# evanwporter/SparseCholesky

Hardware: AMD Instinct MI355X
Metric: numeric-factorization fp64 GFLOP/s (F=sum colcount^2) (higher is better)
Workload: dtype f64

## Files before the change

### sparsecholesky_amd/csrc/kernels.hip

```cpp
#include <hip/hip_runtime.h>

#include <cstdint>
#include <type_traits>

#include "kernels.hpp"

namespace sc {

typedef double double4_t __attribute__((ext_vector_type(4)));

__device__ __forceinline__ void report_fail(int32_t* info, const int32_t* post, int32_t col_internal) {
    atomicMin(info, (post ? post[col_internal] : col_internal) + 1);
}

__device__ __forceinline__ int bnd_at(const int32_t* b, int k, int mbc) {
    const int klo = b[0], khi = b[1];
    return k <= klo ? b[2] : (k >= khi ? mbc : b[2 + k - klo]);
}

__device__ __forceinline__ int lower_bound_i32(const int32_t* a, int n, int v) {
    int lo = 0, hi = n;
    while (lo < hi) {
        int mid = (lo + hi) >> 1;
        if (a[mid] < v)
// ... 947 lines not shown
        if (has_parent) {
            put(i + 1);
            take();
            if (i + 2 < count) prefetch(i + 2);
        }
        if (stamp && tid == 0) stamp[2] = __builtin_amdgcn_s_memtime();
        small_steps<1>(R, colbuf, w, P.info, P.post, d.c0);
        if (w == 0) lds_barrier();
        if (stamp && tid == 0) stamp[3] = __builtin_amdgcn_s_memtime();
        small_store_panel<1>(R, P.panel_pool + d.panel_off, m, w);
        if (m > w && R.bi[0] >= 0 && 4 * R.bi[0] + 3 >= w) {
            if (!has_parent) {
                small_store_cb<1>(R, P.cb_pool + d.cb_off, m, w);
            } else {
                const int mp = ds[i + 1].m;
                double* Fp = Fb(i + 1);
#pragma unroll
                for (int r = 0; r < 4; ++r)
#pragma unroll
                    for (int c = 0; c < 4; ++c) {
                        const int ii = 4 * R.bi[0] + r, jj = 4 * R.bj[0] + c;
                        const int pr = (rr >> (8 * r)) & 255, pc = (rc >> (8 * c)) & 255;
                        if (jj >= w && ii >= jj && ii < m) Fp[pk_col(mp, pc) + pr - pc] += R.v[0][r * 4 + c];
                    }
            }
        }
        lds_barrier();
        if (stamp && tid == 0) stamp[4] = __builtin_amdgcn_s_memtime();
    }
}

#include "panel_gen.inc"

__global__ __launch_bounds__(256) void potrf_tiles_kernel(DevPlan P, const int2* __restrict__ tasks) {
    __shared__ __attribute__((aligned(16))) double colbuf[2 * 4 * COLB];
    const int2 t = tasks[blockIdx.x];
    const int s = t.x, k0 = t.y;
    const int c0 = P.sn_start[s];
    const int w = P.sn_start[s + 1] - c0;
    const int m = P.sn_m[s];
    const int nb = min(PNB, w - k0);
    double* blk = P.panel_pool + P.panel_off[s] + (int64_t)k0 * m + k0;
    SmallRegs<1> R;
    small_tiles<1>(R, nb, nb);
#pragma unroll
    for (int r = 0; r < 4; ++r)
#pragma unroll
        for (int c = 0; c < 4; ++c) {
            const int i = 4 * R.bi[0] + r, j = 4 * R.bj[0] + c;
            R.v[0][r * 4 + c] = (R.bi[0] >= 0 && i < nb && i >= j) ? blk[(int64_t)j * m + i] : 0.0;
        }
    if (SC_POTRF_FAST)
        small_steps1_fast(R, colbuf, nb, P.info, P.post, c0 + k0);
    else
        small_steps<1>(R, colbuf, nb, P.info, P.post, c0 + k0);
    if (R.bi[0] < 0) return;
#pragma unroll
    for (int r = 0; r < 4; ++r)
#pragma unroll
        for (int c = 0; c < 4; ++c) {
            const int i = 4 * R.bi[0] + r, j = 4 * R.bj[0] + c;
            if (i < nb && i >= j) blk[(int64_t)j * m + i] = R.v[0][r * 4 + c];
        }
}

__device__ __forceinline__ void trsm_partial(double* pan, int m, int k0, int nb, int r0, int nrows, double* Lc,
                                             double* invd) {
    constexpr int LD = PNB + 2;
    const int tid = threadIdx.x;
    const double* blk = pan + (int64_t)k0 * m + k0;
    for (int idx = tid; idx < PNB * PNB; idx += TRSM_ROWS) {
        const int q = idx % PNB, j = idx / PNB;
        const double v = (q < nb && j < nb && j <= q) ? blk[(int64_t)j * m + q] : 0.0;
        Lc[j * LD + q] = v;
        if (q == j) invd[j] = (j < nb) ? 1.0 / v : 0.0;
    }
    __syncthreads();
    const int row = r0 + tid;
    const bool live = row < m && tid < nrows;
    double* xs = pan + (int64_t)k0 * m + (live ? row : r0);
    double r[PNB];
#pragma unroll
    for (int c = 0; c < PNB; ++c) r[c] = (live && c < nb) ? xs[(int64_t)c * m] : 0.0;
    trsm_steps<0>(r, Lc, invd, nb);
    if (live) {
#pragma unroll
        for (int c = 0; c < PNB; ++c)
            if (c < nb) xs[(int64_t)c * m] = r[c];
    }
}

__global__ __launch_bounds__(TRSM_ROWS) void trsm_partial_kernel(DevPlan P, const TrsmTask* __restrict__ tasks) {
    __shared__ double Lc[PNB * (PNB + 2)];
    __shared__ double invd[PNB];
    const TrsmTask t = tasks[blockIdx.x];
    const int s = t.s, k0 = t.k0, r0 = t.r0;
    const int c0 = P.sn_start[s];
    const int w = P.sn_start[s + 1] - c0;
    const int m = P.sn_m[s];
    trsm_partial(P.panel_pool + P.panel_off[s], m, k0, min(PNB, w - k0), r0, min(TRSM_ROWS, t.r1 - r0), Lc, invd);
}

template <int PRE>
__global__ __launch_bounds__(TRSM_ROWS) void trsm_panel_g_kernel(DevPlan P, const TrsmTask* __restrict__ tasks,
                                                                 int32_t* __restrict__ arrive) {
    static_assert(TRSM_ROWS == 256, "the fused POTRF maps 4 x 4 tiles onto 256 threads");
    __shared__ double2 S[TRSM64_STREAM / 2];
    __shared__ __attribute__((aligned(16))) double colbuf[2 * 4 * COLB];
    __shared__ int s_last;
    const TrsmTask t = tasks[blockIdx.x];
    const int s = t.s, k0 = t.k0, r0 = t.r0, r1 = t.r1;
    const int tid = threadIdx.x;
    const int c0 = P.sn_start[s];
    const int w = P.sn_start[s + 1] - c0;
    const int m = P.sn_m[s];
    const int nb = min(PNB, w - k0);
    double* pan = P.panel_pool + P.panel_off[s];
    if (nb < PNB) return;
    double* blk = pan + (int64_t)k0 * m + k0;
    double* Sd = reinterpret_cast<double*>(S);
    SmallRegs<1> R;
    small_tiles<1>(R, PNB, PNB);
#pragma unroll
    for (int r = 0; r < 4; ++r)
#pragma unroll
        for (int c = 0; c < 4; ++c) {
            const int i = 4 * R.bi[0] + r, j = 4 * R.bj[0] + c;
            R.v[0][r * 4 + c] = (R.bi[0] >= 0 && i >= j) ? blk[(int64_t)j * m + i] : 0.0;
        }
    if constexpr (PRE == 2) {
        if (R.bi[0] >= 0) {
#pragma unroll
            for (int r = 0; r < 4; ++r)
#pragma unroll
                for (int c = 0; c < 4; ++c) {
                    const int i = 4 * R.bi[0] + r, j = 4 * R.bj[0] + c;
                    if (i >= j) Sd[PNB * j - j * (j - 1) / 2 + (i - j)] = (i == j) ? 1.0 / R.v[0][r * 4 + c] : R.v[0][r * 4 + c];
                }
        }
        const int row = r0 + tid;
        const __amdgpu_buffer_rsrc_t rs = buf_rsrc(pan + (int64_t)k0 * m, (uint32_t)m * PNB * 8u);
        const int voff = row < r1 ? row * 8 : BUF_DEAD;
        double r[PNB];
#pragma unroll
        for (int c = 0; c < PNB; ++c) r[c] = buf_ld(rs, voff, c * m * 8);
        __syncthreads();
        trsm64_full(r, S);
#pragma unroll
        for (int c = 0; c < PNB; ++c) buf_st(r[c], rs, voff, c * m * 8);
        return;
    }
    if (SC_POTRF_FAST)
        small_steps1_fast(R, colbuf, PNB, P.info, P.post, c0 + k0);
    else
        small_steps<1>(R, colbuf, PNB, P.info, P.post, c0 + k0);
    if (R.bi[0] >= 0) {
#pragma unroll
        for (int r = 0; r < 4; ++r)
#pragma unroll
            for (int c = 0; c < 4; ++c) {
                const int i = 4 * R.bi[0] + r, j = 4 * R.bj[0] + c;
                if (i >= j) Sd[PNB * j - j * (j - 1) / 2 + (i - j)] = (i == j) ? 1.0 / R.v[0][r * 4 + c] : R.v[0][r * 4 + c];
            }
    }
    const int row = r0 + tid;
    const __amdgpu_buffer_rsrc_t rs = buf_rsrc(pan + (int64_t)k0 * m, (uint32_t)m * PNB * 8u);
    const int voff = row < r1 ? row * 8 : BUF_DEAD;
    double r[PNB];
#pragma unroll
    for (int c = 0; c < PNB; ++c) r[c] = buf_ld(rs, voff, c * m * 8);
    __syncthreads();
    if (tid == 0) {
        const int k1 = k0 + PNB;
        const int nwg = (max(r1, k1 + 1) - k1 + TRSM_ROWS - 1) / TRSM_ROWS;
        const int old = __hip_atomic_fetch_add(arrive + (t.ctr - 1), 1, __ATOMIC_RELAXED, __HIP_MEMORY_SCOPE_AGENT);
        s_last = old == nwg - 1;
        if (old == nwg - 1) __hip_atomic_store(arrive + (t.ctr - 1), 0, __ATOMIC_RELAXED, __HIP_MEMORY_SCOPE_AGENT);
    }
    __syncthreads();
    if (s_last && R.bi[0] >= 0) {
#pragma unroll
        for (int rr = 0; rr < 4; ++rr)
#pragma unroll
            for (int c = 0; c < 4; ++c) {
                const int i = 4 * R.bi[0] + rr, j = 4 * R.bj[0] + c;
                if (i >= j) blk[(int64_t)j * m + i] = R.v[0][rr * 4 + c];
            }
    }
    trsm64_full(r, S);
#pragma unroll
    for (int c = 0; c < PNB; ++c) buf_st(r[c], rs, voff, c * m * 8);
}

#ifndef SC_PROBE_NOGATHER
#define SC_PROBE_NOGATHER 0
#endif
#ifndef SC_PROBE_NOK
#define SC_PROBE_NOK 0
#endif
template <int BT, int WM, int WN, int BK = 16, int GR = 64>
__device__ __forceinline__ void syrk_gather_epilogue(const GemmTask& T, const int64_t* __restrict__ gblk,
                                                     const GSeg* __restrict__ gseg, int row0, int col0,
                                                     double4_t (&acc)[BT / WM / 16][BT / WN / 16], double* smem) {
    constexpr int NW = WM * WN, NT = 64 * NW;
    constexpr int RTM = BT / WM / 16, RTN = BT / WN / 16;
    constexpr int GLD = GR + 1;
    constexpr int GQ = BT == 64 ? (GR == 32 ? 8 : 64 / NW) : SC_GATHER_Q;
    constexpr int SB = BT == 64 ? 4 : 1;
    constexpr int OPS = 2 * 2 * BK * (BT + 16);
    static_assert(BT * GLD <= OPS, "gather chunk fits the operand LDS");
    const int tid = threadIdx.x, lane = tid & 63, wid = tid >> 6;
    const int wr = wid / WN, wc = wid % WN;
    const int w = T.gw;
    const int mb = T.M;
    const int nb = (mb + 63) >> 6;
    const int64_t* __restrict__ blk = gblk + T.gb;
    const GSeg* __restrict__ seg = gseg;
    double* G = smem;
    double* __restrict__ C = T.C;
    const int64_t ldc = T.ldc;
    const __amdgpu_buffer_rsrc_t rc = buf_rsrc(C + (int64_t)col0 * ldc, (uint32_t)(min(BT, T.N - col0) * ldc * 8));
#pragma unroll 1
    for (int h = 0; h < BT / GR; ++h) {
        const int r0 = row0 + h * GR;
        const int rb = r0 >> 6;
        if (h) __syncthreads();
        for (int e = tid; e < BT * GLD; e += NT) G[e] = 0.0;
        __syncthreads();
        const int cb1 = min(min(nb, rb + 1), (col0 + BT) >> 6);
        for (int cbk = col0 >> 6; !SC_PROBE_NOGATHER && r0 < mb && cbk < cb1; ++cbk) {
            const int64_t bi = (int64_t)rb * (rb + 1) / 2 + cbk;
            const int64_t p0 = blk[bi], p1 = blk[bi + 1];
            for (int64_t pb = p0; pb < p1; pb += SB) {
                int prw[SB], pcl[SB];
#pragma unroll
                for (int q = 0; q < SB; ++q) {
                    prw[q] = -1;
                    pcl[q] = -1;
                    if (pb + q < p1) {
                        const GSeg& g = seg[pb + q];
                        const int ic = g.ilo + lane, jl = g.jlo + lane;
                        if (ic < g.ihi) prw[q] = g.rel[ic] - w - r0;
                        if (jl < g.jhi) pcl[q] = g.rel[jl] - w - col0;
                    }
                }
#pragma unroll
                for (int q = 0; q < SB; ++q) {
                    if (pb + q >= p1) break;
                    const GSeg& g = seg[pb + q];
                    const int ic = g.ilo + lane;
                    const int prow = prw[q] < GR ? prw[q] : -1;
                    const int mbc = g.mbc;
                    const double* __restrict__ cb = g.cb;
                    uint64_t mask = __ballot(pcl[q] >= 0 && pcl[q] % NW == wid);
                    while (mask) {
                        int jc[GQ], pc[GQ];
#pragma unroll
                        for (int u = 0; u < GQ; ++u) {
                            const int b = mask ? __builtin_ctzll(mask) : -1;
                            jc[u] = b < 0 ? -1 : g.jlo + b;
                            pc[u] = b < 0 ? 0 : __builtin_amdgcn_readlane(pcl[q], b);
                            mask &= mask - 1;
                        }
                        double v[GQ];
                        bool ok[GQ];
#pragma unroll
                        for (int u = 0; u < GQ; ++u) {
                            ok[u] = jc[u] >= 0 && prow >= 0 && ic >= jc[u];
                            const __amdgpu_buffer_rsrc_t rs = buf_rsrc(cb + (int64_t)max(jc[u], 0) * mbc, (uint32_t)mbc * 8u);
                            v[u] = buf_ld(rs, ok[u] ? ic * 8 : BUF_DEAD, 0);
                        }
#pragma unroll
                        for (int u = 0; u < GQ; ++u)
                            if (ok[u]) G[pc[u] * GLD + prow] += v[u];
                    }
                }
            }
        }
        __syncthreads();
        static_assert(GR % (BT / WM) == 0, "a wave's rows lie in one chunk");
        if ((wr * (BT / WM)) / GR == h) {
#pragma unroll
            for (int a = 0; a < RTM; ++a)
#pragma unroll
                for (int b = 0; b < RTN; ++b)
#pragma unroll
                    for (int r = 0; r < 4; ++r) {
                        const int lr = wr * (BT / WM) + a * 16 + MFMA_F64_ROW(lane, r);
                        const int lc = wc * (BT / WN) + b * 16 + (lane & 15);
                        G[lc * GLD + (lr - h * GR)] -= acc[a][b][r];
                    }
        }
        __syncthreads();
#pragma unroll 4
        for (int e = tid; e < BT * GR; e += NT) {
            const int lr = e % GR, lc = e / GR;
            const int gi = r0 + lr, gj = col0 + lc;
            const bool live = gi < T.M && gi >= gj && gj < T.N;
            buf_st(G[lc * GLD + lr], rc, live ? (int)((gi + (int64_t)(gj - col0) * ldc) * 8) : BUF_DEAD, 0);
        }
    }
}

template <int BT, int WM, int WN, int BK = 16, int GR = 64>
__device__ __forceinline__ void syrk_rmw_epilogue(const GemmTask& T, int row0, int col0,
                                                  double4_t (&acc)[BT / WM / 16][BT / WN / 16], double* smem) {
    constexpr int NW = WM * WN, NT = 64 * NW;
    constexpr int RTM = BT / WM / 16, RTN = BT / WN / 16;
    constexpr int GLD = GR + 1;
    constexpr int OPS = 2 * 2 * BK * (BT + 16);
    static_assert(BT * GLD <= OPS, "chunk fits the operand LDS");
    static_assert(GR % (BT / WM) == 0, "a wave's rows lie in one chunk");
    const int tid = threadIdx.x, lane = tid & 63, wid = tid >> 6;
    const int wr = wid / WN, wc = wid % WN;
    double* G = smem;
    const int64_t ldc = T.ldc;
    const __amdgpu_buffer_rsrc_t rc = buf_rsrc(T.C + (int64_t)col0 * ldc, (uint32_t)(min(BT, T.N - col0) * ldc * 8));
#pragma unroll 1
    for (int h = 0; h < BT / GR; ++h) {
        const int r0 = row0 + h * GR;
        if (h) __syncthreads();
#pragma unroll 4
        for (int e = tid; e < BT * GR; e += NT) {
            const int lr = e % GR, lc = e / GR;
            const int gi = r0 + lr, gj = col0 + lc;
            const bool live = gi < T.M && gi >= gj && gj < T.N;
            G[lc * GLD + lr] = buf_ld(rc, live ? (int)((gi + (int64_t)(gj - col0) * ldc) * 8) : BUF_DEAD, 0);
        }
        __syncthreads();
        if ((wr * (BT / WM)) / GR == h) {
#pragma unroll
            for (int a = 0; a < RTM; ++a)
#pragma unroll
                for (int b = 0; b < RTN; ++b)
#pragma unroll
                    for (int r = 0; r < 4; ++r) {
                        const int lr = wr * (BT / WM) + a * 16 + MFMA_F64_ROW(lane, r);
                        const int lc = wc * (BT / WN) + b * 16 + (lane & 15);
                        G[lc * GLD + (lr - h * GR)] -= acc[a][b][r];
                    }
        }
        __syncthreads();
#pragma unroll 4
        for (int e = tid; e < BT * GR; e += NT) {
            const int lr = e % GR, lc = e / GR;
            const int gi = r0 + lr, gj = col0 + lc;
            const bool live = gi < T.M && gi >= gj && gj < T.N;
            buf_st(G[lc * GLD + lr], rc, live ? (int)((gi + (int64_t)(gj - col0) * ldc) * 8) : BUF_DEAD, 0);
        }
    }
}

template <int BT, int WM, int WN, int BK = 16>
__device__ __forceinline__ void mfma_kloop(const double* __restrict__ A, int64_t lda, int K, int M, int N, int row0,
                                           int col0, double4_t (&acc)[BT / WM / 16][BT / WN / 16], double* smem) {
    static_assert(BK == 16 || BK == 8, "four-deep k sub-steps of the MFMA");
    constexpr int NT = 64 * WM * WN;
    constexpr int LDT = BT + 16;
    constexpr int RTM = BT / WM / 16, RTN = BT / WN / 16;
    double(*As)[BK * LDT] = reinterpret_cast<double(*)[BK * LDT]>(smem);
    double(*Bs)[BK * LDT] = reinterpret_cast<double(*)[BK * LDT]>(smem + 2 * BK * LDT);
    const int tid = threadIdx.x;
    const int lane = tid & 63;
    const int wid = tid >> 6;
    const int wr = wid / WN, wc = wid % WN;
    constexpr int PER = BT * BK / NT;
    double ra[PER], rb[PER];
    auto gload = [&](int k0) {
        const __amdgpu_buffer_rsrc_t rs = buf_rsrc(A + (int64_t)k0 * lda, (uint32_t)(min(BK, K - k0) * lda * 8));
#pragma unroll
        for (int q = 0; q < PER; ++q) {
            const int e = tid + q * NT;
            const int r = e % BT, kk = e / BT;
            const int gr = row0 + r, gc = col0 + r;
            ra[q] = buf_ld(rs, gr < M ? (int)((gr + kk * lda) * 8) : BUF_DEAD, 0);
            rb[q] = buf_ld(rs, gc < N ? (int)((gc + kk * lda) * 8) : BUF_DEAD, 0);
        }
    };
    auto sstore = [&](int buf) {
#pragma unroll
        for (int q = 0; q < PER; ++q) {
            const int e = tid + q * NT;
            const int r = e % BT, kk = e / BT;
            As[buf][kk * LDT + r] = ra[q];
            Bs[buf][kk * LDT + r] = rb[q];
        }
    };

    const int nk = (K + BK - 1) / BK;
    auto stage = [&](int kt, auto last) {
        constexpr bool LAST = decltype(last)::value;
        const int cur = kt & 1;
        if (!LAST) gload((kt + 1) * BK);
        double av[2][RTM], bv[2][RTN];
        auto lread = [&](int kk, int slot) {
            const int krow = kk + (lane >> 4);
#pragma unroll
            for (int a = 0; a < RTM; ++a)
                av[slot][a] = As[cur][krow * LDT + wr * (BT / WM) + a * 16 + (lane & 15)];
#pragma unroll
            for (int b = 0; b < RTN; ++b)
                bv[slot][b] = Bs[cur][krow * LDT + wc * (BT / WN) + b * 16 + (lane & 15)];
        };
        lread(0, 0);
#pragma unroll
        for (int kk = 0; kk < BK; kk += 4) {
            const int slot = (kk / 4) & 1;
            if (kk + 4 < BK) lread(kk + 4, slot ^ 1);
#pragma unroll
            for (int a = 0; a < RTM; ++a)
#pragma unroll
                for (int b = 0; b < RTN; ++b)
                    acc[a][b] = __builtin_amdgcn_mfma_f64_16x16x4f64(av[slot][a], bv[slot][b], acc[a][b], 0, 0, 0);
            if (!LAST && kk == BK - 8) sstore(cur ^ 1);
        }
        __syncthreads();
    };
    gload(0);
    sstore(0);
    __syncthreads();
    for (int kt = 0; kt + 1 < nk; ++kt) stage(kt, std::false_type {});
    if (nk > 0) stage(nk - 1, std::true_type {});
}

template <int BK>
__device__ __forceinline__ void panel_prefactor(const GemmTask& T, int32_t* info, const int32_t* post,
                                                double* smem) {
    static_assert(2 * 2 * BK * (64 + 16) >= 64 * 65 / 2, "the packed diagonal block fits the operand LDS");
    double4_t acc[2][2];
#pragma unroll
    for (int a = 0; a < 2; ++a)
#pragma unroll
        for (int b = 0; b < 2; ++b) acc[a][b] = (double4_t){0.0, 0.0, 0.0, 0.0};
    mfma_kloop<64, 2, 2, BK>(T.A, T.lda, T.K, T.M, T.N, 0, 0, acc, smem);
    const int tid = threadIdx.x, lane = tid & 63, wid = tid >> 6;
    const int wr = wid >> 1, wc = wid & 1;
    const int64_t ldc = T.ldc;
    double* __restrict__ F = smem;
    const __amdgpu_buffer_rsrc_t rc = buf_rsrc(T.C, (uint32_t)(64 * ldc * 8));
    double cv[2][2][4];
#pragma unroll
    for (int a = 0; a < 2; ++a)
#pragma unroll
        for (int b = 0; b < 2; ++b)
#pragma unroll
            for (int r = 0; r < 4; ++r) {
                const int gi = wr * 32 + a * 16 + MFMA_F64_ROW(lane, r), gj = wc * 32 + b * 16 + (lane & 15);
                cv[a][b][r] = buf_ld(rc, gi >= gj ? (int)((gi + (int64_t)gj * ldc) * 8) : BUF_DEAD, 0);
            }
#pragma unroll
    for (int a = 0; a < 2; ++a)
#pragma unroll
        for (int b = 0; b < 2; ++b)
#pragma unroll
            for (int r = 0; r < 4; ++r) {
                const int gi = wr * 32 + a * 16 + MFMA_F64_ROW(lane, r), gj = wc * 32 + b * 16 + (lane & 15);
                if (gi >= gj) F[pk_col(64, gj) + gi - gj] = cv[a][b][r] - acc[a][b][r];
            }
    __syncthreads();
    SmallRegs<1> R;
    small_tiles<1>(R, PNB, PNB);
    small_load<1>(R, F, PNB);
    __syncthreads();
    small_steps1_fast(R, smem, PNB, info, post, T.pf);
    if (R.bi[0] < 0) return;
#pragma unroll
    for (int r = 0; r < 4; ++r)
#pragma unroll
        for (int c = 0; c < 4; ++c) {
            const int i = 4 * R.bi[0] + r, j = 4 * R.bj[0] + c;
            if (i >= j) T.C[(int64_t)j * ldc + i] = R.v[0][r * 4 + c];
        }
}

template <int BT, int WM, int WN, int TAG, int EPI, int LEAN = 0, int PF = 0>
__device__ __forceinline__ void syrk_tile_body(const GemmTask* __restrict__ tasks, const int2* __restrict__ tiles,
                                               int bidx, const int64_t* __restrict__ gblk,
                                               const GSeg* __restrict__ gseg, int32_t* info = nullptr,
                                               const int32_t* post = nullptr) {
    constexpr int BK = LEAN ? 8 : 16;
    constexpr int LDT = BT + 16;
    constexpr int RTM = BT / WM / 16, RTN = BT / WN / 16;
    __shared__ __attribute__((aligned(16))) double smem[2 * 2 * BK * LDT];

    const int2 tl = tiles[bidx];
    const GemmTask T = tasks[tl.x];
    if constexpr (PF) {
        static_assert(BT == 64 && WM == 2 && WN == 2 && TAG == 0, "pre-factor on 64 x 64 panel-update tiles");
        if (tl.y < 0) {
            panel_prefactor<BK>(T, info, post, smem);
            return;
        }
    }
    const int ti = tl.y >> 16, tj = tl.y & 0xffff;
    const int row0 = ti * BT, col0 = tj * BT;

    const int wid = threadIdx.x >> 6;
    if (wid >= WM * WN / 2) __builtin_amdgcn_s_setprio(1);

    double4_t acc[RTM][RTN];
#pragma unroll
    for (int a = 0; a < RTM; ++a)
#pragma unroll
        for (int b = 0; b < RTN; ++b) acc[a][b] = (double4_t){0.0, 0.0, 0.0, 0.0};
    if (!(SC_PROBE_NOK && TAG == 1 && T.gs >= 0)) mfma_kloop<BT, WM, WN, BK>(T.A, T.lda, T.K, T.M, T.N, row0, col0, acc, smem);

    if constexpr (TAG == 1) {
        if (T.gs >= 0) {
            syrk_gather_epilogue<BT, WM, WN, BK, LEAN ? 32 : 64>(T, gblk, gseg, row0, col0, acc, smem);
            return;
        }
    }
    syrk_rmw_epilogue<BT, WM, WN, BK, LEAN ? 32 : 64>(T, row0, col0, acc, smem);
}

template <int BT, int WM, int WN, int TAG, int EPI, int LEAN = 0, int PF = 0>
__global__ __launch_bounds__(64 * WM * WN, LEAN ? (TAG ? 5 : 6) : 1) void syrk_mfma_kernel(const GemmTask* __restrict__ tasks,
                                                                  const int2* __restrict__ tiles,
                                                                  const int64_t* __restrict__ gblk,
                                                                  const GSeg* __restrict__ gseg, int32_t* info,
                                                                  const int32_t* post) {
    syrk_tile_body<BT, WM, WN, TAG, EPI, LEAN, PF>(tasks, tiles, blockIdx.x, gblk, gseg, info, post);
}

static int small_kt(int maxm) {
    const int T = (maxm + 3) / 4;
    return (T * (T + 1) / 2 + 255) / 256;
}

hipError_t launch_front_small(const DevPlan& P, const int32_t* nodes, int count, int maxm, bool seq,
                              const double* Ax, hipStream_t st) {
    if (count <= 0) return hipSuccess;
    const size_t lds = (size_t)maxm * (maxm + 1) / 2 * sizeof(double);
    const int kt = small_kt(maxm);
    const dim3 grid(seq ? 1 : count);
    const int sq = seq ? count : 0;
    if (kt <= 1)
        hipLaunchKernelGGL(front_small_kernel<1>, grid, dim3(256), lds, st, P, nodes, Ax, sq);
    else if (kt == 2)
        hipLaunchKernelGGL(front_small_kernel<2>, grid, dim3(256), lds, st, P, nodes, Ax, sq);
    else
        hipLaunchKernelGGL(front_small_kernel<3>, grid, dim3(256), lds, st, P, nodes, Ax, sq);
    return hipGetLastError();
}

hipError_t launch_front_chain(const DevPlan& P, const ChainPlan& C, int first, int count, int maxm,
                              const double* Ax, hipStream_t st) {
    if (count <= 0) return hipSuccess;
    if (count > CHAIN_MAXF || maxm > 128) return hipErrorInvalidValue;
    const int fsz = maxm * (maxm + 1) / 2;
    const size_t lds = (size_t)fsz * sizeof(double);
    hipLaunchKernelGGL(chain_init_kernel, dim3(count), dim3(256), lds, st, P, C, first, Ax);
    hipLaunchKernelGGL(front_chain_kernel, dim3(1), dim3(CHAIN_NT), (SC_CHAIN_DB ? 2 : 1) * lds, st, P, C, first, count,
                       fsz);
    return hipGetLastError();
}

hipError_t launch_assemble_large(const DevPlan& P, const int2* tasks, int count, const double* Ax,
                                 hipStream_t st, bool tiled, const int2* lim) {
    if (count <= 0) return hipSuccess;
    if (tiled)
        hipLaunchKernelGGL(assemble_tile_kernel, dim3(count), dim3(256), 0, st, P, tasks, Ax, lim);
    else
        hipLaunchKernelGGL(assemble_cols_kernel, dim3(count), dim3(256), 0, st, P, tasks, Ax);
    return hipGetLastError();
}

hipError_t launch_potrf_diag(const DevPlan& P, const int2* tasks, int count, hipStream_t st) {
    if (count <= 0) return hipSuccess;
    hipLaunchKernelGGL(potrf_tiles_kernel, dim3(count), dim3(256), 0, st, P, tasks);
    return hipGetLastError();
}

hipError_t launch_trsm_panel(const DevPlan& P, const TrsmTask* tasks, int count, hipStream_t st, bool partial,
                             int32_t* arrive, int pre) {
    if (count <= 0) return hipSuccess;
    if (partial)
        hipLaunchKernelGGL(trsm_partial_kernel, dim3(count), dim3(TRSM_ROWS), 0, st, P, tasks);
    else if (pre == 2)
        hipLaunchKernelGGL(trsm_panel_g_kernel<2>, dim3(count), dim3(TRSM_ROWS), 0, st, P, tasks, arrive);
    else
        hipLaunchKernelGGL(trsm_panel_g_kernel<0>, dim3(count), dim3(TRSM_ROWS), 0, st, P, tasks, arrive);
    return hipGetLastError();
}

template <int TAG, int EPI>
static void launch_syrk_t(const GemmTask* tasks, const int2* tiles, int n, int bt, hipStream_t st, GatherTab gt,
                          bool lean) {
    if (bt == 64 && lean)
        hipLaunchKernelGGL((syrk_mfma_kernel<64, 2, 2, TAG, EPI, 1>), dim3(n), dim3(256), 0, st, tasks, tiles, gt.blk,
                           gt.seg, gt.info, gt.post);
    else if (bt == 128)
        hipLaunchKernelGGL((syrk_mfma_kernel<128, 2, 4, TAG, EPI>), dim3(n), dim3(512), 0, st, tasks, tiles, gt.blk,
                           gt.seg, gt.info, gt.post);
    else
        hipLaunchKernelGGL((syrk_mfma_kernel<64, 2, 2, TAG, EPI>), dim3(n), dim3(256), 0, st, tasks, tiles, gt.blk,
                           gt.seg, gt.info, gt.post);
}

hipError_t launch_syrk(const GemmTask* tasks, const int2* tiles, int total_tiles, int bt, int tag, hipStream_t st,
                       int epi, GatherTab gt, bool lean, bool pf) {
    if (total_tiles <= 0) return hipSuccess;
    if (pf) {
        if (bt != 64 || tag) return hipErrorInvalidValue;
        hipLaunchKernelGGL((syrk_mfma_kernel<64, 2, 2, 0, 1, 0, 1>), dim3(total_tiles), dim3(256), 0, st, tasks, tiles,
                           gt.blk, gt.seg, gt.info, gt.post);
        return hipGetLastError();
    }
    if (tag)
        epi ? launch_syrk_t<1, 1>(tasks, tiles, total_tiles, bt, st, gt, lean)
            : launch_syrk_t<1, 0>(tasks, tiles, total_tiles, bt, st, gt, lean);
    else
        epi ? launch_syrk_t<0, 1>(tasks, tiles, total_tiles, bt, st, gt, lean)
            : launch_syrk_t<0, 0>(tasks, tiles, total_tiles, bt, st, gt, lean);
    return hipGetLastError();
}

__global__ void fill_random_kernel(double* p, int64_t n) {
    for (int64_t i = blockIdx.x * (int64_t)blockDim.x + threadIdx.x; i < n; i += (int64_t)gridDim.x * blockDim.x) {
        uint64_t x = (uint64_t)i * 0x9E3779B97F4A7C15ull;
        x ^= x >> 31;
        x *= 0xBF58476D1CE4E5B9ull;
        x ^= x >> 29;
        p[i] = (double)(x >> 11) * (2.0 / 9007199254740992.0) - 1.0;
    }
}

hipError_t launch_fill_random(double* p, int64_t n, hipStream_t st) {
    hipLaunchKernelGGL(fill_random_kernel, dim3(1024), dim3(256), 0, st, p, n);
    return hipGetLastError();
}

__global__ void stamp_kernel(uint64_t* slot) { *slot = __builtin_amdgcn_s_memrealtime(); }

__global__ void status_publish_kernel(int32_t* info, int32_t* host) {
    const int32_t v = __hip_atomic_load(info, __ATOMIC_RELAXED, __HIP_MEMORY_SCOPE_AGENT);
    __hip_atomic_store(info, 0x7f7f7f7f, __ATOMIC_RELAXED, __HIP_MEMORY_SCOPE_AGENT);
    __hip_atomic_store(host, v, __ATOMIC_RELEASE, __HIP_MEMORY_SCOPE_SYSTEM);
}

hipError_t launch_status_publish(int32_t* info, int32_t* host, hipStream_t st) {
    hipLaunchKernelGGL(status_publish_kernel, dim3(1), dim3(1), 0, st, info, host);
    return hipGetLastError();
}

__global__ void hwid_kernel(uint32_t* out, int spin) {
    if (threadIdx.x == 0) {
        out[2 * blockIdx.x] = __builtin_amdgcn_s_getreg((31 << 11) | 4);
        out[2 * blockIdx.x + 1] = __builtin_amdgcn_s_getreg((15 << 11) | 20);
    }
    const uint64_t t0 = __builtin_amdgcn_s_memrealtime();
    while (__builtin_amdgcn_s_memrealtime() - t0 < (uint64_t)spin) __builtin_amdgcn_s_sleep(8);
}

hipError_t launch_hwid(uint32_t* out, int nwg, int threads, int spin, hipStream_t st) {
    hipLaunchKernelGGL(hwid_kernel, dim3(nwg), dim3(threads), 0, st, out, spin);
    return hipGetLastError();
}

hipError_t launch_stamp(uint64_t* slot, hipStream_t st) {
    hipLaunchKernelGGL(stamp_kernel, dim3(1), dim3(1), 0, st, slot);
    return hipGetLastError();
}

__global__ __launch_bounds__(256) void copy2d_kernel(const Copy2D* __restrict__ descs, const int2* __restrict__ tiles,
                                                     int unpack) {
    const int2 t = tiles[blockIdx.x];
    const Copy2D d = descs[t.x];
    const int lane = threadIdx.x & 63, wid = threadIdx.x >> 6;
    const int j0 = t.y & 0xffff, r0 = (t.y >> 16) * COPY_ROWS;
    const int j1 = min(d.cols, j0 + COPY_COLS), r1 = min(d.rows, r0 + COPY_ROWS);
    for (int j = j0 + wid; j < j1; j += 4) {
        const double* __restrict__ src = unpack ? d.b + (int64_t)j * d.rows : d.a + (int64_t)j * d.lda;
        double* __restrict__ dst = unpack ? d.a + (int64_t)j * d.lda : d.b + (int64_t)j * d.rows;
        for (int r = r0 + lane; r < r1; r += 64 * 8) {
            double v[8];
#pragma unroll
            for (int u = 0; u < 8; ++u) v[u] = r + 64 * u < r1 ? src[r + 64 * u] : 0.0;
#pragma unroll
            for (int u = 0; u < 8; ++u)
                if (r + 64 * u < r1) dst[r + 64 * u] = v[u];
        }
    }
}

hipError_t launch_copy2d(const Copy2D* descs, const int2* tiles, int count, bool unpack, hipStream_t st) {
    if (count <= 0) return hipSuccess;
    hipLaunchKernelGGL(copy2d_kernel, dim3(count), dim3(256), 0, st, descs, tiles, unpack ? 1 : 0);
    return hipGetLastError();
}

template <int NACC>
__global__ __launch_bounds__(256) void mfma_peak_kernel(double* out, int iters) {
    double4_t acc[NACC];
#pragma unroll
    for (int j = 0; j < NACC; ++j) acc[j] = (double4_t){0.0, 0.0, 0.0, 0.0};
    const double a = 1.0 + threadIdx.x * 1e-9, b = 1.0 - blockIdx.x * 1e-9;
    for (int i = 0; i < iters; i += 16) {
#pragma unroll
        for (int u = 0; u < 16; ++u)
#pragma unroll
            for (int j = 0; j < NACC; ++j) acc[j] = __builtin_amdgcn_mfma_f64_16x16x4f64(a, b, acc[j], 0, 0, 0);
    }
    double s = 0.0;
#pragma unroll
    for (int j = 0; j < NACC; ++j) s += acc[j][0] + acc[j][1] + acc[j][2] + acc[j][3];
    if (s == 1234.5) out[blockIdx.x] = s;
}

hipError_t launch_mfma_peak(double* out, int blocks, int iters, int nacc, hipStream_t st) {
    if (nacc == 16)
        hipLaunchKernelGGL((mfma_peak_kernel<16>), dim3(blocks), dim3(256), 0, st, out, iters);
    else if (nacc == 8)
        hipLaunchKernelGGL((mfma_peak_kernel<8>), dim3(blocks), dim3(256), 0, st, out, iters);
    else if (nacc == 2)
        hipLaunchKernelGGL((mfma_peak_kernel<2>), dim3(blocks), dim3(256), 0, st, out, iters);
    else
        hipLaunchKernelGGL((mfma_peak_kernel<4>), dim3(blocks), dim3(256), 0, st, out, iters);
    return hipGetLastError();
}

__global__ __launch_bounds__(64) void solve_inv_kernel(SolvePlan P, const int2* __restrict__ tasks) {
    __shared__ double2 S[TRSM64_STREAM / 2];
    __shared__ double Lc[PNB * (PNB + 2)];
    __shared__ double invd[PNB];
    const int2 t = tasks[blockIdx.x];
    const int s = t.x, k0 = t.y;
    const int lane = threadIdx.x;
    const int c0 = P.sn_start[s];
    const int w = P.sn_start[s + 1] - c0;
    const int m = P.sn_m[s];
    const int nb = min(PNB, w - k0);
    double* blk = const_cast<double*>(P.panel_pool) + P.panel_off[s] + (int64_t)k0 * m + k0;
    double r[PNB];
    {
#pragma unroll
        for (int j = 0; j < PNB; ++j) r[j] = (j < nb && lane < nb && lane >= j) ? blk[(int64_t)j * m + lane] : 0.0;
    }
    if (nb == PNB) {
        double* Sd = reinterpret_cast<double*>(S);
#pragma unroll
        for (int j = 0; j < PNB; ++j)
            if (lane >= j) Sd[PNB * j - j * (j - 1) / 2 + (lane - j)] = lane == j ? 1.0 / r[j] : r[j];
    } else {
        constexpr int LD = PNB + 2;
#pragma unroll
        for (int j = 0; j < PNB; ++j) {
            Lc[j * LD + lane] = r[j];
            if (lane == j) invd[j] = j < nb ? 1.0 / r[j] : 0.0;
        }
    }
    __syncthreads();
#pragma unroll
    for (int c = 0; c < PNB; ++c) r[c] = c == lane ? 1.0 : 0.0;
    if (nb == PNB)
        trsm64_full(r, S);
    else
        trsm_steps<0>(r, Lc, invd, nb);
#pragma unroll
    for (int c = 0; c < PNB; ++c)
        if (lane < c && c < nb) blk[(int64_t)c * m + lane] = r[c];
}

__global__ __launch_bounds__(256) void solve_inv2_kernel(SolvePlan P, const int2* __restrict__ tasks) {
    __shared__ double Xa[PNB][PNB + 1], Bm[PNB][PNB + 1], Xb[PNB][PNB + 1];
    const int2 t = tasks[blockIdx.x];
    const int s = t.x, k0 = t.y;
    const int tid = threadIdx.x;
    const int c0 = P.sn_start[s];
    const int w = P.sn_start[s + 1] - c0;
    const int m = P.sn_m[s];
    const int nbb = min(SOLVE_NB, w - k0) - PNB;
    double* blk = const_cast<double*>(P.panel_pool) + P.panel_off[s] + (int64_t)k0 * m + k0;
    const double* blkb = blk + (int64_t)PNB * m + PNB;
#pragma unroll
    for (int q = 0; q < PNB * PNB / 256; ++q) {
        const int e = tid + 256 * q, i = e >> 6, k = e & 63;
        Xa[i][k] = k < i ? blk[(int64_t)i * m + k] : (k == i ? 1.0 / blk[(int64_t)i * m + i] : 0.0);
        Xb[i][k] = (i < nbb && k < i) ? blkb[(int64_t)i * m + k] : ((i < nbb && k == i) ? 1.0 / blkb[(int64_t)i * m + i] : 0.0);
        Bm[k][i] = k < nbb ? blk[(int64_t)i * m + PNB + k] : 0.0;
    }
    __syncthreads();
    const int i = tid >> 2, jg = tid & 3;
    double acc[16];
#pragma unroll
    for (int q = 0; q < 16; ++q) acc[q] = 0.0;
    for (int k = 0; k < PNB; ++k) {
        const double bik = Bm[i][k];
#pragma unroll
        for (int q = 0; q < 16; ++q) acc[q] = fma(bik, Xa[k][jg + 4 * q], acc[q]);
    }
    __syncthreads();
#pragma unroll
    for (int q = 0; q < 16; ++q) Bm[i][jg + 4 * q] = acc[q];
    __syncthreads();
#pragma unroll
    for (int q = 0; q < 16; ++q) acc[q] = 0.0;
    for (int k = 0; k <= i; ++k) {
        const double xik = Xb[i][k];
#pragma unroll
        for (int q = 0; q < 16; ++q) acc[q] = fma(xik, Bm[k][jg + 4 * q], acc[q]);
    }
    if (i < nbb) {
#pragma unroll
        for (int q = 0; q < 16; ++q) blk[(int64_t)(PNB + i) * m + jg + 4 * q] = -acc[q];
    }
}

__device__ __forceinline__ void quad_apply(const double* __restrict__ blk, int64_t m, int nb, int I, int K,
                                           const double* cb, double* out, bool add, double (*part)[PNB],
                                           double (*Xs)[PNB + 1]) {
    const int tid = threadIdx.x;
    const __amdgpu_buffer_rsrc_t rs = buf_rsrc(blk, (uint32_t)(((int64_t)(nb - 1) * m + nb) * 8));
    double v[PNB * PNB / 256];
#pragma unroll
    for (int q = 0; q < PNB * PNB / 256; ++q) {
        const int e = tid + 256 * q, i = e >> 6, k = e & 63;
        const int gi = PNB * I + i, gk = PNB * K + k;
        v[q] = buf_ld(rs, (gi < nb && gk <= gi) ? (int)(((int64_t)gi * m + gk) * 8) : BUF_DEAD, 0);
    }
// ... 1113 lines not shown
```

Baseline: 56850.

## Prefetch C tile before k-loop and simplify RMW epilogue addressing

Restructures the SYRK read-modify-write epilogue so each lane keeps a fixed row and steps through columns with precomputed buffer offsets and a per-lane column limit, replacing per-element index math and liveness checks. For 64-wide non-lean update tiles, the first chunk of C is loaded into registers before the MFMA k-loop so the global load latency overlaps the compute. The next chunk is loaded before the barrier. Launch-bound occupancy hints are also raised. This trades more live registers during the k-loop for hidden load latency and cheaper addressing.

New measurement: 57120, median of 6. Within noise of the previous version (+0.5%).

```diff
diff --git a/sparsecholesky_amd/csrc/kernels.hip b/sparsecholesky_amd/csrc/kernels.hip
--- a/sparsecholesky_amd/csrc/kernels.hip
+++ b/sparsecholesky_amd/csrc/kernels.hip
@@ -1273,31 +1273,60 @@
     }
 }
 
+template <int BT, int NT, int GR>
+struct RmwLane {
+    static constexpr int CS = NT / GR, NQ = BT / CS;
+    static_assert(NT % GR == 0 && BT % CS == 0, "a lane keeps its row; whole column steps");
+    __amdgpu_buffer_rsrc_t rc;
+    int sstep;
+    int voff0;
+    int mrow;
+    int ncl;
+    int drow;
+
+    __device__ __forceinline__ RmwLane(const GemmTask& T, int row0, int col0) {
+        const int tid = threadIdx.x, lr = tid % GR, lc0 = tid / GR;
+        const int ldc = (int)T.ldc;
+        const int ncol = min(BT, T.N - col0);
+        rc = buf_rsrc(T.C + (int64_t)col0 * ldc, (uint32_t)(ncol * ldc * 8));
+        sstep = CS * ldc * 8;
+        voff0 = (row0 + lr + lc0 * ldc) * 8;
+        mrow = T.M - (row0 + lr);
+        ncl = ncol - 1 - lc0;
+        drow = row0 >= col0 + BT ? 2 * BT : row0 + lr - col0 - lc0;
+    }
+    __device__ __forceinline__ int voff(int h) const { return voff0 + h * GR * 8; }
+    __device__ __forceinline__ int qlim(int h) const { return h * GR < mrow ? min(ncl, drow + h * GR) : -1; }
+    __device__ __forceinline__ void load(int h, double (&v)[NQ]) const {
+        const int vo = voff(h), ql = qlim(h);
+#pragma unroll
+        for (int q = 0; q < NQ; ++q) v[q] = buf_ld(rc, q * CS <= ql ? vo : BUF_DEAD, q * sstep);
+    }
+};
+
 template <int BT, int WM, int WN, int BK = 16, int GR = 64>
-__device__ __forceinline__ void syrk_rmw_epilogue(const GemmTask& T, int row0, int col0,
+__device__ __forceinline__ void syrk_rmw_epilogue(const RmwLane<BT, 64 * WM * WN, GR>& L,
+                                                  double (&cv)[RmwLane<BT, 64 * WM * WN, GR>::NQ],
                                                   double4_t (&acc)[BT / WM / 16][BT / WN / 16], double* smem) {
     constexpr int NW = WM * WN, NT = 64 * NW;
     constexpr int RTM = BT / WM / 16, RTN = BT / WN / 16;
     constexpr int GLD = GR + 1;
     constexpr int OPS = 2 * 2 * BK * (BT + 16);
+    constexpr int CS = NT / GR, NQ = BT / CS;
     static_assert(BT * GLD <= OPS, "chunk fits the operand LDS");
     static_assert(GR % (BT / WM) == 0, "a wave's rows lie in one chunk");
     const int tid = threadIdx.x, lane = tid & 63, wid = tid >> 6;
     const int wr = wid / WN, wc = wid % WN;
     double* G = smem;
-    const int64_t ldc = T.ldc;
-    const __amdgpu_buffer_rsrc_t rc = buf_rsrc(T.C + (int64_t)col0 * ldc, (uint32_t)(min(BT, T.N - col0) * ldc * 8));
-#pragma unroll 1
+    double* Gl = G + (tid / GR) * GLD + tid % GR;
+#pragma unroll
     for (int h = 0; h < BT / GR; ++h) {
-        const int r0 = row0 + h * GR;
-        if (h) __syncthreads();
-#pragma unroll 4
-        for (int e = tid; e < BT * GR; e += NT) {
-            const int lr = e % GR, lc = e / GR;
-            const int gi = r0 + lr, gj = col0 + lc;
-            const bool live = gi < T.M && gi >= gj && gj < T.N;
-            G[lc * GLD + lr] = buf_ld(rc, live ? (int)((gi + (int64_t)(gj - col0) * ldc) * 8) : BUF_DEAD, 0);
-        }
+        if (h) {
+            L.load(h, cv);
+            __syncthreads();
+        }
+#pragma unroll
+        for (int q = 0; q < NQ; ++q) Gl[q * CS * GLD] = cv[q];
         __syncthreads();
         if ((wr * (BT / WM)) / GR == h) {
 #pragma unroll
@@ -1312,13 +1341,9 @@
                     }
         }
         __syncthreads();
-#pragma unroll 4
-        for (int e = tid; e < BT * GR; e += NT) {
-            const int lr = e % GR, lc = e / GR;
-            const int gi = r0 + lr, gj = col0 + lc;
-            const bool live = gi < T.M && gi >= gj && gj < T.N;
-            buf_st(G[lc * GLD + lr], rc, live ? (int)((gi + (int64_t)(gj - col0) * ldc) * 8) : BUF_DEAD, 0);
-        }
+        const int vo = L.voff(h), ql = L.qlim(h);
+#pragma unroll
+        for (int q = 0; q < NQ; ++q) buf_st(Gl[q * CS * GLD], L.rc, q * CS <= ql ? vo : BUF_DEAD, q * L.sstep);
     }
 }
 
@@ -1474,6 +1499,11 @@
     for (int a = 0; a < RTM; ++a)
 #pragma unroll
         for (int b = 0; b < RTN; ++b) acc[a][b] = (double4_t){0.0, 0.0, 0.0, 0.0};
+    constexpr bool CPRE = TAG == 0 && BT == 64 && !LEAN;
+    using Lane = RmwLane<BT, 64 * WM * WN, LEAN ? 32 : 64>;
+    double cv[Lane::NQ];
+    if constexpr (CPRE) Lane(T, row0, col0).load(0, cv);
+
     if (!(SC_PROBE_NOK && TAG == 1 && T.gs >= 0)) mfma_kloop<BT, WM, WN, BK>(T.A, T.lda, T.K, T.M, T.N, row0, col0, acc, smem);
 
     if constexpr (TAG == 1) {
@@ -1482,11 +1512,13 @@
             return;
         }
     }
-    syrk_rmw_epilogue<BT, WM, WN, BK, LEAN ? 32 : 64>(T, row0, col0, acc, smem);
+    const Lane L(T, row0, col0);
+    if constexpr (!CPRE) L.load(0, cv);
+    syrk_rmw_epilogue<BT, WM, WN, BK, LEAN ? 32 : 64>(L, cv, acc, smem);
 }
 
 template <int BT, int WM, int WN, int TAG, int EPI, int LEAN = 0, int PF = 0>
-__global__ __launch_bounds__(64 * WM * WN, LEAN ? (TAG ? 5 : 6) : 1) void syrk_mfma_kernel(const GemmTask* __restrict__ tasks,
+__global__ __launch_bounds__(64 * WM * WN, LEAN ? (TAG ? 6 : 7) : PF ? 3 : 4) void syrk_mfma_kernel(const GemmTask* __restrict__ tasks,
                                                                   const int2* __restrict__ tiles,
                                                                   const int64_t* __restrict__ gblk,
                                                                   const GSeg* __restrict__ gseg, int32_t* info,
```
